# acoustic-warfare/beamforming-lk

Measured on AMD Instinct MI355X. Metric: heatmap frames/sec, higher is better.
Workload: dtype f32

## Files before the change

beamforming-lk_amd/csrc/das_fast.hip:

```cpp
#include "das_kernels.h"

#include <algorithm>
#include <atomic>

namespace awpu {

typedef float f2 __attribute__((ext_vector_type(2)));
typedef float f4 __attribute__((ext_vector_type(4)));
typedef float f4u __attribute__((ext_vector_type(4), aligned(4)));
typedef float f8 __attribute__((ext_vector_type(8)));

#define AWPU_AS4 __attribute__((address_space(4)))

typedef int i16 __attribute__((ext_vector_type(16)));

struct EntryGroup {
    i16 v;
    __device__ __forceinline__ float f(int k) const { return __int_as_float(v[4 * k + 0]); }
    __device__ __forceinline__ unsigned addr(int k) const { return (unsigned) v[4 * k + 1]; }
    __device__ __forceinline__ float g(int k) const { return __int_as_float(v[4 * k + 2]); }
};

template <int FPI>
struct Reads {
// ... 39 lines not shown
    issue_reads<FPI>(r1, e.addr(1), lane_base);
    issue_reads<FPI>(r2, e.addr(2), lane_base);
    issue_reads<FPI>(r3, e.addr(3), lane_base);
    accumulate<FPI>(acc, r0, e.f(0), e.g(0));
    accumulate<FPI>(acc, r1, e.f(1), e.g(1));
    accumulate<FPI>(acc, r2, e.f(2), e.g(2));
    accumulate<FPI>(acc, r3, e.f(3), e.g(3));
}

#include "das_fast_trip.inc"
static_assert(kFirStaticPlaneBytes == kFirStaticPlaneBytesHost, "das_kernels.h and tools/gen_trip_asm.py disagree on the FIR8 plane pitch");

template <int PPW, bool LOW = false>
__device__ __forceinline__ void sweep_chunk_trips(Acc<1> (&acc)[PPW], const FastEntry *lut, int pix0,
                                                  int usable_pad, int m0, int ng, unsigned lane_addr) {
    const int stride = usable_pad * (int) sizeof(FastEntry);
    if constexpr (PPW % 4 == 0 && LOW) {
#pragma unroll
        for (int q = 0; q < PPW; q += 4) {
            const void *row = lut + (size_t) (pix0 + q) * usable_pad + m0;
            sweep_quad_lo(acc[q].A[0], acc[q].Q[0], acc[q].C[0], acc[q].R[0],
                          acc[q + 1].A[0], acc[q + 1].Q[0], acc[q + 1].C[0], acc[q + 1].R[0],
                          acc[q + 2].A[0], acc[q + 2].Q[0], acc[q + 2].C[0], acc[q + 2].R[0],
                          acc[q + 3].A[0], acc[q + 3].Q[0], acc[q + 3].C[0], acc[q + 3].R[0], row, stride, ng, lane_addr);
        }
    } else if constexpr (PPW % 4 == 0) {
#pragma unroll
        for (int q = 0; q < PPW; q += 4) {
            const void *row = lut + (size_t) (pix0 + q) * usable_pad + m0;
            sweep_quad_hi(acc[q].A[0], acc[q].Q[0], acc[q].C[0], acc[q].R[0],
                          acc[q + 1].A[0], acc[q + 1].Q[0], acc[q + 1].C[0], acc[q + 1].R[0],
                          acc[q + 2].A[0], acc[q + 2].Q[0], acc[q + 2].C[0], acc[q + 2].R[0],
                          acc[q + 3].A[0], acc[q + 3].Q[0], acc[q + 3].C[0], acc[q + 3].R[0], row, stride, ng, lane_addr);
        }
    } else {
#pragma unroll
        for (int pp = 0; pp < PPW; pp++) {
            const void *row = lut + (size_t) (pix0 + pp) * usable_pad + m0;
            sweep_pixel_hi(acc[pp].A[0], acc[pp].Q[0], acc[pp].C[0], acc[pp].R[0], row, stride, ng, lane_addr);
        }
    }
}

template <int PPW, bool LOW = false>
__device__ __forceinline__ void sweep_chunk_stamped(Acc<1> (&acc)[PPW], const FastEntry *lut, int pix0,
                                                    int usable_pad, int m0, int ng, unsigned lane_addr,
                                                    unsigned &t_wait, unsigned &t_all) {
    static_assert(PPW % 4 == 0, "diagnostic build: quads only");
    const int stride = usable_pad * (int) sizeof(FastEntry);
#pragma unroll
    for (int q = 0; q < PPW; q += 4) {
        const void *row = lut + (size_t) (pix0 + q) * usable_pad + m0;
        unsigned dw = 0, da = 0;
        if constexpr (LOW) {
            sweep_quad_lo_stamped(acc[q].A[0], acc[q].Q[0], acc[q].C[0], acc[q].R[0],
                                  acc[q + 1].A[0], acc[q + 1].Q[0], acc[q + 1].C[0], acc[q + 1].R[0],
                                  acc[q + 2].A[0], acc[q + 2].Q[0], acc[q + 2].C[0], acc[q + 2].R[0],
                                  acc[q + 3].A[0], acc[q + 3].Q[0], acc[q + 3].C[0], acc[q + 3].R[0], row, stride, ng,
                                  lane_addr, dw, da);
        } else
        sweep_quad_stamped(acc[q].A[0], acc[q].Q[0], acc[q].C[0], acc[q].R[0],
                           acc[q + 1].A[0], acc[q + 1].Q[0], acc[q + 1].C[0], acc[q + 1].R[0],
                           acc[q + 2].A[0], acc[q + 2].Q[0], acc[q + 2].C[0], acc[q + 2].R[0],
                           acc[q + 3].A[0], acc[q + 3].Q[0], acc[q + 3].C[0], acc[q + 3].R[0], row, stride, ng,
                           lane_addr, dw, da);
        t_wait += dw;
        t_all += da;
    }
}

template <int CTRL, int ROW_MASK = 0xf>
__device__ __forceinline__ float dpp_take(float v) {
    return __builtin_bit_cast(float, __builtin_amdgcn_update_dpp(0, __builtin_bit_cast(int, v), CTRL, ROW_MASK, 0xf, false));
}
__device__ __forceinline__ float wave_sum(float v) {
    v += dpp_take<0xB1>(v);
    v += dpp_take<0x4E>(v);
    v += dpp_take<0x141>(v);
    v += dpp_take<0x140>(v);
    v += dpp_take<0x142, 0xa>(v);
    v += dpp_take<0x143, 0xc>(v);
    return __builtin_bit_cast(float, __builtin_amdgcn_readlane(__builtin_bit_cast(int, v), 63));
}

__device__ __forceinline__ float fold_halves(float a, float b) {
    asm volatile("s_nop 1\n\tv_permlane32_swap_b32 %0, %1\n\ts_nop 1" : "+v"(a), "+v"(b));
    return a + b;
}
__device__ __forceinline__ float fold_rows(float a, float b) {
    asm volatile("s_nop 1\n\tv_permlane16_swap_b32 %0, %1\n\ts_nop 1" : "+v"(a), "+v"(b));
    return a + b;
}
__device__ __forceinline__ float wave_sum8(float v0, float v1, float v2, float v3, float v4, float v5, float v6, float v7, int lane) {
    const float x = fold_rows(fold_halves(v0, v1), fold_halves(v2, v3));
    const float y = fold_rows(fold_halves(v4, v5), fold_halves(v6, v7));
    const float xs = x + dpp_take<0x128>(x), ys = y + dpp_take<0x128>(y);
    float z = (lane & 8) ? ys : xs;
    z += dpp_take<0xB1>(z);
    z += dpp_take<0x4E>(z);
    z += dpp_take<0x141>(z);
    return z;
}
__device__ __forceinline__ constexpr int kWaveSum8Value(int group) { return 4 * (group & 1) + (((group >> 1) & 1) << 1) + (group >> 2); }
__device__ __forceinline__ float wave_sum4(float v0, float v1, float v2, float v3) {
    float z = fold_rows(fold_halves(v0, v1), fold_halves(v2, v3));
    z += dpp_take<0xB1>(z);
    z += dpp_take<0x4E>(z);
    z += dpp_take<0x141>(z);
    z += dpp_take<0x140>(z);
    return z;
}
__device__ __forceinline__ constexpr int kWaveSum4Value(int row) { return ((row & 1) << 1) + (row >> 1); }

__device__ __forceinline__ void store_powers8(const f2 (&s)[4], const int (&pix)[4], const bool (&live)[4], int pair, int batch,
                                              int pixel_count, float norm, float *power, int lane) {
    const float total = wave_sum8(s[0].x, s[0].y, s[1].x, s[1].y, s[2].x, s[2].y, s[3].x, s[3].y, lane);
    const int value = kWaveSum8Value(lane >> 3), pp = value >> 1, frame = 2 * pair + (value & 1);
    const int p = pp == 0 ? pix[0] : pp == 1 ? pix[1] : pp == 2 ? pix[2] : pix[3];
    const bool on = pp == 0 ? live[0] : pp == 1 ? live[1] : pp == 2 ? live[2] : live[3];
    if ((lane & 7) == 0 && on && frame < batch) power[(size_t) frame * pixel_count + p] = total / norm;
}

__device__ __forceinline__ float sum8(float v) {
    v += dpp_take<0xB1>(v);
    v += dpp_take<0x4E>(v);
    v += dpp_take<0x141>(v);
    return v;
}
__device__ __forceinline__ float sum16(float v) {
    v = sum8(v);
    return v + dpp_take<0x140>(v);
}
__device__ __forceinline__ float sum32(float v) {
    v = sum16(v);
    return v + dpp_take<0x142, 0xa>(v);
}
template <int LPP>
__device__ __forceinline__ float sum_lanes(float v) {
    static_assert(LPP == 8 || LPP == 16 || LPP == 32, "groups of 8, 16 or 32 lanes");
    return LPP == 8 ? sum8(v) : LPP == 16 ? sum16(v) : sum32(v);
}
template <int LPP>
__device__ __forceinline__ constexpr int sum_lane_of(int group) {
    return LPP == 32 ? 32 * group + 16 : LPP * group;
}
__device__ __forceinline__ float lane_value(float v, int lane_index) {
    return __builtin_bit_cast(float, __builtin_amdgcn_readlane(__builtin_bit_cast(int, v), lane_index));
}

constexpr int kDppWaveRol1 = 0x134;
constexpr int kDppWaveRor1 = 0x13C;
template <int CTRL>
__device__ __forceinline__ float wave_rotate1(float v) {
    const int bits = __builtin_bit_cast(int, v);
    return __builtin_bit_cast(float, __builtin_amdgcn_update_dpp(bits, bits, CTRL, 0xf, 0xf, false));
}

__device__ __forceinline__ float finish_pixel(f2 A, f2 Q, f2 C, f2 R, float tail, int lane) {
    const float q_rot = wave_rotate1<kDppWaveRol1>(Q.x);
    const float r_rot = wave_rotate1<kDppWaveRol1>(R.x);
    const float q_next = lane == 63 ? r_rot : q_rot;
    const float r_next = lane == 63 ? tail : r_rot;
    const float o0 = A.x + Q.y;
    const float o1 = A.y + q_next;
    const float o2 = C.x + R.y;
    const float o3 = C.y + r_next;
    const float o1_prev = wave_rotate1<kDppWaveRor1>(o1);
    const float o2_next = wave_rotate1<kDppWaveRol1>(o2);
    const float o0_rot = wave_rotate1<kDppWaveRol1>(o0);
    const float o3_rot = wave_rotate1<kDppWaveRor1>(o3);
    const float o0_next = lane == 63 ? o2_next : o0_rot;
    const float o3_prev = lane == 0 ? o1_prev : o3_rot;
    const float ma0 = o0 * 0.5f - 0.25f * (o1 + o1_prev);
    const float ma1 = o1 * 0.5f - 0.25f * (o0_next + o0);
    const float ma2 = o2 * 0.5f - 0.25f * (o3 + o3_prev);
    const float ma3 = o3 * 0.5f - 0.25f * (o2_next + o2);
    float sum = ma1 * ma1 + ma2 * ma2;
    if (lane != 0) sum += ma0 * ma0;
    if (lane != 63) sum += ma3 * ma3;
    return wave_sum(sum);
}

template <int NW, int PPW, int FPI, int WPS>
__global__ __launch_bounds__(NW * 64, WPS) void das_fast_kernel(FastArgs a) {
    static_assert(PPW <= 8, "the tail pass gives 8 lanes to each of at most 8 pixels");
    extern __shared__ __attribute__((aligned(16))) float lds[];
    constexpr int FS = kFastLdsBytes / FPI;
    const int lane = threadIdx.x & 63;
    const int wave = __builtin_amdgcn_readfirstlane(threadIdx.x >> 6);
    const char *lane_base = (const char *) lds + lane * 8;
    const unsigned lane_addr = (unsigned) (unsigned long long) (const __attribute__((address_space(3))) char *) lane_base;
    const int frame0 = blockIdx.x * FPI;
    const int pix0 = (blockIdx.y * NW + wave) * PPW;
    const int wr = a.wr;
    const AWPU_AS4 FastEntry *lut = (const AWPU_AS4 FastEntry *) (unsigned long long) a.lut;
    const AWPU_AS4 int32_t *index = (const AWPU_AS4 int32_t *) (unsigned long long) a.index;
    const AWPU_AS4 int32_t *row_off = (const AWPU_AS4 int32_t *) (unsigned long long) a.row_off;

    Acc<FPI> acc[PPW];
    float tail[FPI];
#pragma unroll
    for (int b = 0; b < FPI; b++) tail[b] = 0.0f;
#pragma unroll
    for (int pp = 0; pp < PPW; pp++)
#pragma unroll
        for (int b = 0; b < FPI; b++) acc[pp].A[b] = acc[pp].Q[b] = acc[pp].C[b] = acc[pp].R[b] = f2{0.0f, 0.0f};

    constexpr int LPP = 8, NU = 32 / LPP;
    const int tail_pp = lane / LPP;
    const bool tail_lane = tail_pp < PPW && pix0 + tail_pp < a.pixel_count;
    const FastEntry *tail_row = a.lut + (size_t) (pix0 + (tail_lane ? tail_pp : 0)) * a.usable_pad;
    struct AddrG {
        unsigned addr;
        float g;
    };

    for (int m0 = 0; m0 < a.usable; m0 += a.chunk) {
        const int mc = min(a.chunk, a.usable - m0);
        const int mc4 = (mc + 3) & ~3;
        AddrG te[NU];
#pragma unroll
        for (int u = 0; u < NU; u++) {
            const int j = LPP * u + ((lane - m0) & (LPP - 1));
            te[u] = *(const AddrG *) ((const char *) (tail_row + m0 + min(j, mc4 - 1)) + 4);
            if (!tail_lane || j >= mc4) te[u].g = 0.0f;
        }
        __syncthreads();

        const int rows = AWPU_DBG(a, 1) && m0 > 0 ? 0 : FPI * mc * 2;
        const bool inside = a.wstart + 1 + wr <= a.hist;
        if (inside && !AWPU_DBG(a, 64)) {
            for (int r = wave; r < rows; r += NW) {
                const int b = r / (2 * mc);
                const int jr = r - b * 2 * mc;
                const int fb = min(frame0 + b, a.batch - 1);
                const float *src = a.frames + (size_t) fb * a.n_streams * a.hist + row_off[2 * m0 + jr];
                float *dst = lds + b * (FS / 4) + jr * wr;
                for (int t0 = 0; t0 < wr; t0 += 256) {
                    if (t0 + lane * 4 < wr) {
                        __builtin_amdgcn_global_load_lds((const __attribute__((address_space(1))) void *) (src + t0 + lane * 4),
                                                         (__attribute__((address_space(3))) void *) (dst + t0), 16, 0, 0);
                    }
                }
            }
            asm volatile("s_waitcnt vmcnt(0)" ::: "memory");
        } else
        for (int r = wave; r < rows; r += 2 * NW) {
            const float *src[2];
            float *dst[2];
            int valid[2];
#pragma unroll
            for (int u = 0; u < 2; u++) {
                const int rr = min(r + u * NW, rows - 1);
                const int b = rr / (2 * mc);
                const int jr = rr - b * 2 * mc;
                const int j = jr >> 1, q = jr & 1;
                const int fb = min(frame0 + b, a.batch - 1);
                const int first = a.wstart + q;
                src[u] = a.frames + ((size_t) fb * a.n_streams + index[m0 + j]) * a.hist + first;
                dst[u] = lds + b * (FS / 4) + (j * 2 + q) * wr;
                valid[u] = min(wr, a.hist - first);
            }
            if (valid[0] == wr && valid[1] == wr) {
                for (int t0 = 0; t0 < wr; t0 += 512) {
                    f4 v[2][2];
#pragma unroll
                    for (int u = 0; u < 2; u++)
#pragma unroll
                        for (int k = 0; k < 2; k++) {
                            const int t = t0 + k * 256 + lane * 4;
                            if (t < wr) v[u][k] = *(const f4u *) (src[u] + t);
                        }
#pragma unroll
                    for (int u = 0; u < 2; u++)
#pragma unroll
                        for (int k = 0; k < 2; k++) {
                            const int t = t0 + k * 256 + lane * 4;
                            if (t < wr) *(f4 *) (dst[u] + t) = v[u][k];
                        }
                }
            } else {
#pragma unroll
                for (int u = 0; u < 2; u++)
                    for (int t = lane; t < wr; t += 64) dst[u][t] = t < valid[u] ? src[u][t] : 0.0f;
            }
        }
        __syncthreads();

        if (!AWPU_DBG(a, 2)) {
            if constexpr (FPI == 1) {
                sweep_chunk_trips<PPW>(acc, a.lut, pix0, a.usable_pad, m0, mc4 >> 2, lane_addr);
            } else {
#pragma unroll
                for (int pp = 0; pp < PPW; pp++) {
                    const int p = pix0 + pp;
                    if (p < a.pixel_count) {
                        const AWPU_AS4 i16 *grp = (const AWPU_AS4 i16 *) (lut + (size_t) p * a.usable_pad + m0);
                        const int ng = mc4 >> 2;
                        EntryGroup e0, e1;
                        e0.v = grp[0];
                        for (int g = 0; g < ng; g += 2) {
                            e1.v = grp[g + 1];
                            sweep_group<FPI>(acc[pp], e0, lane_base);
                            e0.v = grp[g + 2];
                            if (g + 1 < ng) sweep_group<FPI>(acc[pp], e1, lane_base);
                        }
                    }
                }
// ... 119 lines not shown
        const int buf = step & 1;
        const bool last_chunk = c + 1 == n_chunks;
        const int c1 = last_chunk ? 0 : c + 1;
        const int fi1 = last_chunk ? fi + 1 : fi;
        long long t = diag ? __builtin_readcyclecounter() : 0;
        if (step + 1 < n_steps && !AWPU_DBG(a, 1)) {
            dma_chunk(frame0 + fi1, c1 * a.chunk, min(a.chunk, a.usable - c1 * a.chunk), buf ^ 1);
        }
        stamp(0, t);

        const unsigned lane_addr = lds_base + buf * BUF + lane * 8;
        if constexpr (DIAG) {
            sweep_chunk_stamped<PPW, (WPS > 4)>(acc, a.lut, pix0, a.usable_pad, m0, mc4 >> 2, lane_addr, t_wait, t_all);
        } else if (!AWPU_DBG(a, 2)) {
            sweep_chunk_trips<PPW, (WPS > 4)>(acc, a.lut, pix0, a.usable_pad, m0, mc4 >> 2, lane_addr);
        }
        stamp(1, t);
        const float *buf_f = lds + buf * (BUF / 4);
        for (int j0 = 0; j0 < (AWPU_DBG(a, 4) ? 0 : mc4); j0 += 32) {
            FastEntry e[4];
#pragma unroll
            for (int u = 0; u < 4; u++) {
                const int j = j0 + 8 * u + ((lane - m0) & 7);
                e[u] = tail_row[m0 + min(j, mc4 - 1)];
                if (!tail_lane || j >= mc4) e[u].g = 0.0f;
            }
#pragma unroll
            for (int u = 0; u < 4; u++) tail = __builtin_fmaf(e[u].g, buf_f[(e[u].addr + 1024u) >> 2], tail);
        }
        if (diag) asm volatile("s_waitcnt lgkmcnt(0)" ::: "memory");
        stamp(2, t);
        asm volatile("s_waitcnt vmcnt(0)" ::: "memory");
        stamp(3, t);
        if (!AWPU_DBG(a, 8)) __syncthreads();
        stamp(4, t);

        if (last_chunk) {
            tail = sum8(tail);
#pragma unroll
            for (int pp = 0; pp < PPW; pp++) {
                const int p = pix0 + pp;
                const float tl = lane_value(tail, pp * 8);
                const float sum = finish_pixel(acc[pp].A[0], acc[pp].Q[0], acc[pp].C[0], acc[pp].R[0], tl, lane);
                if (lane == 0 && p < a.pixel_count) {
                    a.power[(size_t) (frame0 + fi) * a.pixel_count + p] = sum / (float) (kSamples * a.usable);
                }
                acc[pp].A[0] = acc[pp].Q[0] = acc[pp].C[0] = acc[pp].R[0] = f2{0.0f, 0.0f};
            }
            tail = 0.0f;
        }
        c = c1;
        fi = fi1;
    }

    if (DIAG && a.debug_out && lane == 0) {
        unsigned long long *o = a.debug_out + 12 * ((size_t) (blockIdx.y * gridDim.x + blockIdx.x) * NW + wave);
        o[0] = t_wait;
        o[1] = t_all;
        o[2] = (unsigned long long) (__builtin_readcyclecounter() - t_begin);
        o[3] = (unsigned long long) n_steps * PPW;
        for (int k = 0; k < 5; k++) o[4 + k] = t_ph[k];
    }
}

template <bool FILTER>
__device__ __forceinline__ void pack_one_row(const float *frames, int n_streams, int hist, int wstart, const int32_t *index,
                                             int usable, const float *gain, int wp, int batch, float *packed, int pair, int s,
                                             int rows_out) {
    f2 *dst = (f2 *) packed + ((size_t) pair * rows_out + s) * wp;
    if (s >= usable) {
        for (int t = threadIdx.x; t < wp; t += blockDim.x) dst[t] = f2{0.0f, 0.0f};
        return;
    }
    const int fa = min(2 * pair, batch - 1), fb = min(2 * pair + 1, batch - 1);
    const float *xa = frames + ((size_t) fa * n_streams + index[s]) * hist + wstart;
    const float *xb = frames + ((size_t) fb * n_streams + index[s]) * hist + wstart;
    const float gm = gain ? gain[s] : 1.0f;
    const int valid = min(wp, hist - wstart);
    for (int t = threadIdx.x; t < wp; t += blockDim.x) {
        f2 v = f2{0.0f, 0.0f};
        if (t < valid) {
            v = f2{xa[t] * gm, xb[t] * gm};
            if constexpr (FILTER) {
                const bool lo = wstart + t > 0, hi = wstart + t + 1 < hist;
                const f2 nb = f2{(lo ? xa[t - 1] * gm : 0.0f) + (hi ? xa[t + 1] * gm : 0.0f),
                                 (lo ? xb[t - 1] * gm : 0.0f) + (hi ? xb[t + 1] * gm : 0.0f)};
                v = __builtin_elementwise_fma(f2{-0.25f, -0.25f}, nb, 0.5f * v);
            }
        }
        dst[t] = v;
    }
}

template <bool FILTER>
__global__ void pack_pairs_kernel(const float *frames, int n_streams, int hist, int wstart, const int32_t *index,
                                  int usable, const float *gain, int wp, int batch, float *packed) {
    pack_one_row<FILTER>(frames, n_streams, hist, wstart, index, usable, gain, wp, batch, packed, blockIdx.y, blockIdx.x, gridDim.x);
}

template <int CTRL>
__device__ __forceinline__ f2 wave_rotate(f2 v) {
    return f2{wave_rotate1<CTRL>(v.x), wave_rotate1<CTRL>(v.y)};
}

__device__ __forceinline__ f2 finish_pixel_pair(const f2 (&P)[8], f2 tail, int lane) {
    f2 o[4];
    f2 rq = wave_rotate<kDppWaveRol1>(P[4]);
#pragma unroll
    for (int k = 0; k < 4; k++) {
        const f2 rq_next = k < 3 ? wave_rotate<kDppWaveRol1>(P[k < 3 ? 5 + k : 7]) : tail;
        o[k] = P[k] + (lane == 63 ? rq_next : rq);
        rq = rq_next;
    }
    f2 sum = f2{0.0f, 0.0f};
    f2 dn = wave_rotate<kDppWaveRol1>(o[0]);
    f2 up_before = wave_rotate<kDppWaveRor1>(o[0]);
#pragma unroll
    for (int k = 0; k < 4; k++) {
        const f2 dn_after = k < 3 ? wave_rotate<kDppWaveRol1>(o[k < 3 ? k + 1 : 3]) : dn;
        const f2 up = wave_rotate<kDppWaveRor1>(o[k]);
        const f2 next = lane == 63 ? dn_after : dn;
        const f2 prev = lane == 0 ? up_before : up;
        const int i = lane + 64 * k;
        const f2 ma = o[k] * 0.5f - 0.25f * (next + prev);
        if (i >= 1 && i <= kSamples - 2) sum += ma * ma;
        dn = dn_after;
        up_before = up;
    }
    sum.x = wave_sum(sum.x);
    sum.y = wave_sum(sum.y);
    return sum;
}

__device__ __forceinline__ f2 pixel_pair_partial_filtered(const f2 (&P)[8], int lane) {
    f2 sum = f2{0.0f, 0.0f};
    f2 rq = wave_rotate<kDppWaveRol1>(P[4]);
#pragma unroll
    for (int k = 0; k < 4; k++) {
        const f2 rq_next = k < 3 ? wave_rotate<kDppWaveRol1>(P[k < 3 ? 5 + k : 7]) : rq;
        const f2 ma = P[k] + (lane == 63 ? rq_next : rq);
        const int i = lane + 64 * k;
        if (i >= 1 && i <= kSamples - 2) sum = __builtin_elementwise_fma(ma, ma, sum);
        rq = rq_next;
    }
    return sum;
}
__device__ __forceinline__ f2 finish_pixel_pair_filtered(const f2 (&P)[8], int lane) {
    f2 sum = pixel_pair_partial_filtered(P, lane);
    sum.x = wave_sum(sum.x);
    sum.y = wave_sum(sum.y);
    return sum;
}

__device__ __forceinline__ const void *uniform_ptr(const void *p) {
    const unsigned long long v = (unsigned long long) p;
    const unsigned lo = __builtin_amdgcn_readfirstlane((unsigned) v);
    const unsigned hi = __builtin_amdgcn_readfirstlane((unsigned) (v >> 32));
    return (const void *) (((unsigned long long) hi << 32) | lo);
}

template <int PPW, bool DIAG, bool SHARE>
__global__ __launch_bounds__(1024, 4) void das_pair_kernel(PairArgs a) {
    static_assert(PPW % 2 == 0 && PPW <= 8, "pixels go through the asm blocks two at a time");
    extern __shared__ __attribute__((aligned(16))) float lds[];
    constexpr int NW = 16, kThreads = NW * 64, BUF = kFastLdsBytes;
    constexpr int kPieces = (BUF + kThreads * 16 - 1) / (kThreads * 16);
    const int lane = threadIdx.x & 63;
    const int wave = __builtin_amdgcn_readfirstlane(threadIdx.x >> 6);
    const unsigned lds_base = (unsigned) (unsigned long long) (const __attribute__((address_space(3))) char *) lds;
    const int total = a.n_pairs * a.tiles;
    const int per_xcd = (total + 7) >> 3;
    const int item = (blockIdx.x & 7) * per_xcd + (blockIdx.x >> 3);
    if (item >= min(total, ((int) (blockIdx.x & 7) + 1) * per_xcd)) return;
    int pair, tile;
    {
        const int full_items = (a.n_pairs / a.pair_group) * a.pair_group * a.tiles;
        const int ga = item < full_items ? a.pair_group : a.n_pairs % a.pair_group;
        const int rem = item < full_items ? item : item - full_items;
        const int grp = rem / (a.tiles * ga), in = rem - grp * a.tiles * ga;
        tile = in / ga;
        pair = (item < full_items ? grp * a.pair_group : a.n_pairs - ga) + (in - tile * ga);
    }
    int pix[PPW];
    bool live[PPW];
    int pair_rows;
    if (a.cols > 0) {
        static_assert(PPW == 4, "vertical pairing: 2 columns x 2 rows per wave");
        const int tiles_per_rowpair = (a.cols + 2 * NW - 1) / (2 * NW);
        const int row2 = tile / tiles_per_rowpair, col0 = (tile - row2 * tiles_per_rowpair) * 2 * NW + 2 * wave;
        const int rows = a.pixel_count / a.cols;
#pragma unroll
        for (int q = 0; q < PPW; q++) {
            const int row = 2 * row2 + (q & 1), col = col0 + (q >> 1);
            live[q] = row < rows && col < a.cols;
            pix[q] = min(2 * row2 * a.cols + col, a.pixel_count - 1) + (q & 1) * a.cols;
        }
        pair_rows = a.cols;
    } else {
#pragma unroll
        for (int q = 0; q < PPW; q++) {
            pix[q] = (tile * NW + wave) * PPW + q;
            live[q] = pix[q] < a.pixel_count;
        }
        pair_rows = 1;
    }
    const size_t row_floats = (size_t) a.wp * 2;
    const float *pair_base = a.packed + (size_t) pair * a.usable * row_floats;

    f2 acc[PPW][8];
#pragma unroll
    for (int pp = 0; pp < PPW; pp++)
#pragma unroll
        for (int k = 0; k < 8; k++) acc[pp][k] = f2{0.0f, 0.0f};

    auto dma_chunk = [&](int m0, int mc, int buf) {
        const float *src = pair_base + (size_t) m0 * row_floats;
        const int n_pieces = (int) ((size_t) mc * row_floats / 4);
#pragma unroll
        for (int k = 0; k < kPieces; k++) {
            const int piece = threadIdx.x + k * kThreads;
            if (piece < n_pieces) {
                float *dst = lds + buf * (BUF / 4) + (wave * 64 + k * kThreads) * 4;
                __builtin_amdgcn_global_load_lds((const __attribute__((address_space(1))) void *) (src + (size_t) piece * 4),
                                                 (__attribute__((address_space(3))) void *) dst, 16, 0, 0);
            }
        }
    };

    unsigned t_wait = 0, t_all = 0;
    const long long t_begin = __builtin_readcyclecounter();
    const int n_chunks = (a.usable + a.chunk - 1) / a.chunk;
    dma_chunk(0, min(a.chunk, a.usable), 0);
    asm volatile("s_waitcnt vmcnt(0)" ::: "memory");
    __syncthreads();

    unsigned t_ph[5] = {0, 0, 0, 0, 0};
    auto stamp = [&](int k, long long &t) {
        if (DIAG) {
            const long long n = __builtin_readcyclecounter();
            t_ph[k] += (unsigned) (n - t);
            t = n;
        }
    };
    const int stride = pair_rows * a.usable_pad * (int) sizeof(FastEntry);
    const int rank = wave >> 2;
    for (int c = 0; c < n_chunks; c++) {
        const int m0 = c * a.chunk;
        const int mc = min(a.chunk, a.usable - m0);
        const int mc4 = (mc + 3) & ~3;
        const int buf = c & 1;
        long long t = DIAG ? __builtin_readcyclecounter() : 0;
        if (c + 1 < n_chunks && !AWPU_DBG(a, 1)) dma_chunk(m0 + a.chunk, min(a.chunk, a.usable - m0 - a.chunk), buf ^ 1);
        stamp(0, t);
        const unsigned lane_addr = lds_base + buf * BUF + lane * 8;
#pragma unroll
        for (int q = 0; q < PPW; q += 2) {
            const void *row = uniform_ptr(a.lut + (size_t) pix[q] * a.usable_pad + m0);
            const int ng = __builtin_amdgcn_readfirstlane(mc4 >> 2);
            if constexpr (DIAG) {
                unsigned dw = 0, da = 0;
                if constexpr (SHARE) sweep_duo_shared_stamped(acc[q], acc[q + 1], row, stride, ng, lane_addr, rank, dw, da);
                else sweep_duo_pairs_stamped(acc[q], acc[q + 1], row, stride, ng, lane_addr, rank, dw, da);
                t_wait += dw;
                t_all += da;
            } else {
                if constexpr (SHARE) sweep_duo_shared(acc[q], acc[q + 1], row, stride, ng, lane_addr, rank);
                else sweep_duo_pairs(acc[q], acc[q + 1], row, stride, ng, lane_addr, rank);
            }
        }
        stamp(1, t);
        if (DIAG) asm volatile("s_waitcnt lgkmcnt(0)" ::: "memory");
        stamp(2, t);
        asm volatile("s_waitcnt vmcnt(0)" ::: "memory");
        stamp(3, t);
        if (!AWPU_DBG(a, 8)) __syncthreads();
        stamp(4, t);
    }

    if (DIAG && a.debug_out && lane == 0) {
        unsigned long long *o = a.debug_out + 12 * ((size_t) item * NW + wave);
        o[0] = t_wait;
        o[1] = t_all;
        o[2] = (unsigned long long) (__builtin_readcyclecounter() - t_begin);
        o[3] = (unsigned long long) n_chunks * PPW;
        for (int k = 0; k < 5; k++) o[4 + k] = t_ph[k];
    }
    const float norm = (float) (kSamples * a.usable);
    static_assert(PPW == 4, "store_powers8: four pixels x two frames per wave");
    f2 part[PPW];
#pragma unroll
    for (int pp = 0; pp < PPW; pp++) {
        part[pp] = pixel_pair_partial_filtered(acc[pp], lane);
    }
    store_powers8(part, pix, live, pair, a.batch, a.pixel_count, norm, a.power, lane);
}


template <bool SHARE>
__global__ __launch_bounds__(1024, 4) void das_pair_stationary_kernel(PairArgs a, int n_tiles, int tiles_per_wg) {
    constexpr int PPW = 4;
    extern __shared__ __attribute__((aligned(16))) float lds[];
    constexpr int NW = 16, kThreads = NW * 64;
    const int lane = threadIdx.x & 63;
    const int wave = __builtin_amdgcn_readfirstlane(threadIdx.x >> 6);
    const unsigned lds_base = (unsigned) (unsigned long long) (const __attribute__((address_space(3))) char *) lds;
    const int pair = blockIdx.x;
// ... 251 lines not shown
    const float *pair_base = a.packed + (size_t) pair * a.usable_pad * row_floats;

    f8 O0 = {0, 0, 0, 0, 0, 0, 0, 0}, O1 = O0, O2 = O0, O3 = O0;

    auto dma_chunk = [&](int m0, int mc, int buf) {
        const float *src = pair_base + (size_t) m0 * row_floats;
        const int n_pieces = (int) ((size_t) mc * row_floats / 4);
#pragma unroll
        for (int k = 0; k < kPieces; k++) {
            const int piece = threadIdx.x + k * kThreads;
            if (piece < n_pieces) {
                float *dst = lds + buf * (BUF / 4) + (wave * 64 + k * kThreads) * 4;
                __builtin_amdgcn_global_load_lds((const __attribute__((address_space(1))) void *) (src + (size_t) piece * 4),
                                                 (__attribute__((address_space(3))) void *) dst, 16, 0, 0);
            }
        }
    };

    const int n_chunks = (a.usable_pad + a.chunk - 1) / a.chunk;
    dma_chunk(0, min(a.chunk, a.usable_pad), 0);
    asm volatile("s_waitcnt vmcnt(0)" ::: "memory");
    __syncthreads();
    const int rank = wave >> 2;
    for (int c = 0; c < n_chunks; c++) {
        const int m0 = c * a.chunk;
        const int mc = min(a.chunk, a.usable_pad - m0);
        const int buf = c & 1;
        if (c + 1 < n_chunks) dma_chunk(m0 + a.chunk, min(a.chunk, a.usable_pad - m0 - a.chunk), buf ^ 1);
        const unsigned lane_addr = lds_base + buf * BUF + lane * 8;
        const void *row = uniform_ptr(quad_lut + (size_t) (m0 >> 2) * 16);
        sweep_quad_exact(O0, O1, O2, O3, row, __builtin_amdgcn_readfirstlane(mc >> 2), lane_addr, rank);
        asm volatile("s_waitcnt vmcnt(0)" ::: "memory");
        __syncthreads();
    }

    const float norm = (float) (kSamples * a.usable);
    auto finish = [&](const f8 &O, int q) {
        const int row = 4 * row4 + q;
        const bool live = row < a.rows && col < a.cols;
        const int p = min(row, a.rows - 1) * a.cols + min(col, a.cols - 1);
        f2 o[4];
#pragma unroll
        for (int k = 0; k < 4; k++) o[k] = f2{O[2 * k], O[2 * k + 1]};
        if (a.sums && live) {
#pragma unroll
            for (int k = 0; k < 4; k++) {
                a.sums[((size_t) (2 * pair) * a.pixel_count + p) * kSamples + lane + 64 * k] = o[k].x;
                if (2 * pair + 1 < a.batch) a.sums[((size_t) (2 * pair + 1) * a.pixel_count + p) * kSamples + lane + 64 * k] = o[k].y;
            }
        }
        return pixel_pair_partial_exact(o, lane);
    };
    const f2 s0 = finish(O0, 0), s1 = finish(O1, 1), s2 = finish(O2, 2), s3 = finish(O3, 3);
    {
        const float total = wave_sum8(s0.x, s0.y, s1.x, s1.y, s2.x, s2.y, s3.x, s3.y, lane);
        const int value = kWaveSum8Value(lane >> 3), row = 4 * row4 + (value >> 1), frame = 2 * pair + (value & 1);
        if ((lane & 7) == 0 && row < a.rows && col < a.cols && frame < a.batch)
            a.power[(size_t) frame * a.pixel_count + (size_t) row * a.cols + col] = total / norm;
    }
}

__device__ __forceinline__ f2 next_and_difference(float cur, float next, float gm) {
#pragma clang fp contract(off)
    const float c = cur * gm, n = next * gm;
    return f2{n, c - n};
}

__global__ void pack_nd_kernel(const float *frames, int n_streams, int hist, int wstart, const int32_t *index, int usable,
                               const float *gain, int wq, int batch, float *packed) {
    const int pair = blockIdx.y, s = blockIdx.x, rows_out = gridDim.x;
    f4 *dst = (f4 *) packed + ((size_t) pair * rows_out + s) * wq;
    if (s >= usable) {
        for (int t = threadIdx.x; t < wq; t += blockDim.x) dst[t] = f4{0.0f, 0.0f, 0.0f, 0.0f};
        return;
    }
    const int fa = min(2 * pair, batch - 1), fb = min(2 * pair + 1, batch - 1);
    const float *xa = frames + ((size_t) fa * n_streams + index[s]) * hist + wstart;
    const float *xb = frames + ((size_t) fb * n_streams + index[s]) * hist + wstart;
    const float gm = gain ? gain[s] : 1.0f;
    const int valid = min(wq, hist - wstart - 1);
    for (int t = threadIdx.x; t < wq; t += blockDim.x) {
        f4 v = f4{0.0f, 0.0f, 0.0f, 0.0f};
        if (t < valid) {
            const f2 ea = next_and_difference(xa[t], xa[t + 1], gm), eb = next_and_difference(xb[t], xb[t + 1], gm);
            v = f4{ea.x, eb.x, ea.y, eb.y};
        }
        dst[t] = v;
    }
}

__global__ void nd_items_kernel(int2 *items, int n_pairs, int tiles, int pair_group, int tiles_per_row, int nq) {
    const int item = blockIdx.x * blockDim.x + threadIdx.x;
    if (item >= n_pairs * tiles) return;
    const int full_items = (n_pairs / pair_group) * pair_group * tiles;
    const int ga = item < full_items ? pair_group : n_pairs % pair_group;
    const int rem = item < full_items ? item : item - full_items;
    const int grp = rem / (tiles * ga), in = rem - grp * tiles * ga;
    const int tile = in / ga;
    const int pair = (item < full_items ? grp * pair_group : n_pairs - ga) + (in - tile * ga);
    const int rowq = tile / tiles_per_row, colt = tile - rowq * tiles_per_row;
    items[item] = int2{pair, (nq * rowq * tiles_per_row + colt) * 16};
}

struct NdQueues {
    unsigned *q;
    int per, total, tail;
    __device__ __forceinline__ int len(int x) const { return max(0, min(per, total - x * per)); }
    __device__ __forceinline__ int head(int x) const { return len(x) - min(len(x), tail); }
    __device__ __forceinline__ int take_head(int x) const {
        if (head(x) <= 0) return -1;
        const unsigned i = atomicAdd(&q[x], 1u);
        return i < (unsigned) head(x) ? x * per + (int) i : -1;
    }
    __device__ __forceinline__ int take_common() const {
        if (tail <= 0) return -1;
        for (;;) {
            const unsigned j = atomicAdd(&q[8], 1u);
            const int run = (int) (j / (unsigned) tail), k = (int) (j - (unsigned) run * (unsigned) tail);
            if (run >= 8) return -1;
            if (k < len(run) - head(run)) return run * per + head(run) + k;
        }
    }
    __device__ __forceinline__ int take(int xcd) const {
        int item = take_head(xcd);
        if (item < 0) item = take_common();
        for (int y = 1; item < 0 && y < 8; y++) item = take_head((xcd + y) & 7);
        return item;
    }
};

template <int NQ, bool SUMS>
__global__ __launch_bounds__(1024, 4) void das_exact_nd_kernel(ExactNdArgs a) {
    extern __shared__ __attribute__((aligned(16))) float lds[];
    constexpr int NW = 16, kThreads = NW * 64, BUF = kFastLdsBytes;
    constexpr int kPieces = (BUF + kThreads * 16 - 1) / (kThreads * 16);
    const int wave = __builtin_amdgcn_readfirstlane(threadIdx.x >> 6);
    const unsigned lds_base = (unsigned) (unsigned long long) (const __attribute__((address_space(3))) char *) lds;
    int *mail = (int *) (lds + 2 * (BUF / 4));
    const int total = a.n_pairs * a.tiles;
    unsigned xcc;
    asm volatile("s_getreg_b32 %0, hwreg(HW_REG_XCC_ID)" : "=s"(xcc));
    const NdQueues Q{a.queue, (total + 7) >> 3, total, a.tail};
    const int xcd = (int) (xcc & 7u);
    if (threadIdx.x == 0) {
        const int first = Q.take(xcd);
        mail[0] = first;
        mail[1] = first >= 0 ? Q.take(xcd) : -1;
    }
    __syncthreads();
    int cur = __builtin_amdgcn_readfirstlane(mail[0]), nxt = __builtin_amdgcn_readfirstlane(mail[1]);
    if (cur < 0) return;
    __syncthreads();

    auto decode = [&](int item, int &pair, int &tile_quad) {
        const int2 d = a.items[item];
        pair = __builtin_amdgcn_readfirstlane(d.x);
        tile_quad = __builtin_amdgcn_readfirstlane(d.y);
    };
    const int tiles_per_row = (a.cols + NW - 1) / NW;
    const int groups_total = a.usable_pad >> 2;
    const size_t row_floats = (size_t) a.wq * 4;
    const int n_chunks = (a.usable_pad + a.chunk - 1) / a.chunk;
    const int first_mics = min(a.chunk, a.usable_pad), last_mics = a.usable_pad - (n_chunks - 1) * a.chunk;
    const int ngf = __builtin_amdgcn_readfirstlane(first_mics >> 2), ngl = __builtin_amdgcn_readfirstlane(last_mics >> 2);
    const unsigned dbf = __builtin_amdgcn_readfirstlane((unsigned) ((size_t) a.chunk * row_floats * 4));
    const unsigned dbl = __builtin_amdgcn_readfirstlane((unsigned) ((size_t) last_mics * row_floats * 4));
    const unsigned db0 = __builtin_amdgcn_readfirstlane((unsigned) ((size_t) first_mics * row_floats * 4));
    const int rank = wave >> 2;
    const int own_head = Q.head(xcd);

    int pair, tile;
    decode(cur, pair, tile);
#ifdef AWPU_TUNING_BUILD
    const unsigned long long rt_begin = a.debug_out ? __builtin_amdgcn_s_memrealtime() : 0ull;
    long long t_sweep = 0, t_other = 0, t_mark = __builtin_readcyclecounter();
    int n_items = 0;
#endif
    {
        const float *pair_base = a.packed + (size_t) pair * a.usable_pad * row_floats;
        const int n_pieces = (int) ((size_t) first_mics * row_floats / 4);
#pragma unroll
        for (int k = 0; k < kPieces; k++) {
            const int piece = threadIdx.x + k * kThreads;
            if (piece < n_pieces) {
                float *dst = lds + (wave * 64 + k * kThreads) * 4;
                __builtin_amdgcn_global_load_lds((const __attribute__((address_space(1))) void *) (pair_base + (size_t) piece * 4),
                                                 (__attribute__((address_space(3))) void *) dst, 16, 0, 0);
            }
        }
    }
    asm volatile("s_waitcnt vmcnt(0)" ::: "memory");
    __syncthreads();
    unsigned step = 0;

    for (;;) {
        const int cols_pad = tiles_per_row * NW;
        const int rowq = tile / (NQ * cols_pad);
        const int col = tile - NQ * rowq * cols_pad + wave;
        const int quad0 = tile + wave;
        const QuadEntry *quad_lut = a.lut + (size_t) quad0 * groups_total * 16;
        const float *pair_base = a.packed + (size_t) pair * a.usable_pad * row_floats;
        int pair_next = pair, tile_next = tile;
        if (nxt >= 0) decode(nxt, pair_next, tile_next);
        const float *next_base = a.packed + (size_t) pair_next * a.usable_pad * row_floats;
        unsigned ticket = 0;
        const bool asked = wave == 0 && nxt >= 0 && own_head > 0;
        const unsigned *qptr = (const unsigned *) uniform_ptr(asked ? a.queue + xcd : nullptr);

        f8 O[NQ][4];
#ifdef AWPU_TUNING_BUILD
        { const long long n = __builtin_readcyclecounter(); t_other += n - t_mark; t_mark = n; }
#endif
        {
            unsigned tid = threadIdx.x;
            asm volatile("" : "+v"(tid));
            const unsigned lane_bytes = tid * 16;
            const int buf = (int) (step & 1);
            unsigned lane_addr = lds_base + buf * BUF + (tid & 63) * 16;
            const unsigned ddst = __builtin_amdgcn_readfirstlane(lds_base + (buf ^ 1) * BUF + wave * 1024);
            const int delta = __builtin_amdgcn_readfirstlane(buf ? -BUF : BUF);
            const unsigned dbn = __builtin_amdgcn_readfirstlane(nxt >= 0 ? db0 : 0u);
            if constexpr (NQ == 1) {
                sweep_exact_nd_item1(O[0][0], O[0][1], O[0][2], O[0][3], uniform_ptr(quad_lut), ngf, ngl, __builtin_amdgcn_readfirstlane(n_chunks),
                                     lane_addr, rank, uniform_ptr(pair_base), dbf, dbl, uniform_ptr(next_base), dbn, ddst, delta, lane_bytes, qptr, ticket);
            } else {
                static_assert(NQ == 2, "blocks are generated for one and two quads per wave");
                const int qstride = __builtin_amdgcn_readfirstlane(tiles_per_row * NW * groups_total * 16 * (int) sizeof(QuadEntry));
                sweep_exact_nd_item2(O[0][0], O[0][1], O[0][2], O[0][3], O[1][0], O[1][1], O[1][2], O[1][3], uniform_ptr(quad_lut), qstride, ngf, ngl,
                                     __builtin_amdgcn_readfirstlane(n_chunks), lane_addr, rank, uniform_ptr(pair_base), dbf, dbl, uniform_ptr(next_base),
                                     dbn, ddst, delta, lane_bytes, qptr, ticket);
            }
            step += n_chunks;
        }
        if (threadIdx.x == 0 && nxt >= 0) {
            int got = own_head > 0 && ticket < (unsigned) own_head ? xcd * Q.per + (int) ticket : -1;
            if (got < 0) {
                got = Q.take_common();
                for (int y = 1; got < 0 && y < 8; y++) got = Q.take_head((xcd + y) & 7);
            }
            mail[0] = got;
        }
#ifdef AWPU_TUNING_BUILD
        { const long long n = __builtin_readcyclecounter(); t_sweep += n - t_mark; t_mark = n; n_items++; }
#endif

        unsigned tid_e = threadIdx.x;
        asm volatile("" : "+v"(tid_e));
        const int lane = (int) (tid_e & 63);
        const float norm = (float) (kSamples * a.usable);
#pragma unroll
        for (int q = 0; q < NQ; q++) {
            const int row4 = NQ * rowq + q;
            auto finish = [&](const f8 &Op, int pp) {
                const int row = 4 * row4 + pp;
                const bool live = row < a.rows && col < a.cols;
                const int p = min(row, a.rows - 1) * a.cols + min(col, a.cols - 1);
                f2 o[4];
#pragma unroll
                for (int k = 0; k < 4; k++) o[k] = f2{Op[2 * k], Op[2 * k + 1]};
                if (SUMS && live) {
#pragma unroll
                    for (int k = 0; k < 4; k++) {
                        a.sums[((size_t) (2 * pair) * a.pixel_count + p) * kSamples + lane + 64 * k] = o[k].x;
                        if (2 * pair + 1 < a.batch) a.sums[((size_t) (2 * pair + 1) * a.pixel_count + p) * kSamples + lane + 64 * k] = o[k].y;
                    }
                }
                return pixel_pair_partial_exact(o, lane);
            };
            const f2 s0 = finish(O[q][0], 0), s1 = finish(O[q][1], 1), s2 = finish(O[q][2], 2), s3 = finish(O[q][3], 3);
            const float sum = wave_sum8(s0.x, s0.y, s1.x, s1.y, s2.x, s2.y, s3.x, s3.y, lane);
            const int value = kWaveSum8Value(lane >> 3), row = 4 * row4 + (value >> 1), frame = 2 * pair + (value & 1);
            if ((lane & 7) == 0 && row < a.rows && col < a.cols && frame < a.batch)
                a.power[(size_t) frame * a.pixel_count + (size_t) row * a.cols + col] = sum / norm;
        }

        if (nxt < 0) break;
        __syncthreads();
        cur = nxt;
        pair = pair_next;
        tile = tile_next;
        nxt = __builtin_amdgcn_readfirstlane(mail[0]);
        __syncthreads();
    }
#ifdef AWPU_TUNING_BUILD
    if (a.debug_out && threadIdx.x == 0) {
        unsigned hw_id;
        asm volatile("s_getreg_b32 %0, hwreg(HW_REG_HW_ID)" : "=s"(hw_id));
        unsigned long long *o = a.debug_out + 8 * (size_t) blockIdx.x;
        o[0] = rt_begin;
        o[1] = __builtin_amdgcn_s_memrealtime();
        o[2] = (unsigned long long) t_other;
        o[3] = (unsigned long long) t_sweep;
        o[4] = (unsigned long long) (__builtin_readcyclecounter() - t_mark);
        o[5] = ((unsigned long long) xcc << 32) | hw_id;
        o[6] = (unsigned long long) n_items;
        o[7] = 1;
    }
#endif
}

__device__ __forceinline__ void store_tile_and_signal(float *lds, bool holder, int tile_row, int wave, int lane, float value, float *power, int row0,
                                                      int col0, int rows, int cols, const DoneFlag &done) {
    __syncthreads();
    if (holder) lds[tile_row * 16 + wave] = value;
    __syncthreads();
    if (wave != 0) return;
    const int r = row0 + (lane >> 4), c = col0 + (lane & 15);
    if (r < rows && c < cols) __hip_atomic_store(&power[(size_t) r * cols + c], lds[lane], __ATOMIC_RELAXED, __HIP_MEMORY_SCOPE_SYSTEM);
    asm volatile("s_waitcnt vmcnt(0)" ::: "memory");
    if (lane == 0 && __hip_atomic_fetch_add(done.counter, 1ull, __ATOMIC_RELAXED, __HIP_MEMORY_SCOPE_AGENT) + 1ull == done.target)
        __hip_atomic_store(done.flag, done.seq, __ATOMIC_RELAXED, __HIP_MEMORY_SCOPE_SYSTEM);
}

__global__ void pack_ndh_kernel(const float *frames, int n_streams, int pitch, int wstart, const int32_t *index, int usable,
                                const float *gain, int wh, float *packed) {
    const int frame = blockIdx.y, s = blockIdx.x, rows_out = gridDim.x;
    f4 *dst = (f4 *) packed + ((size_t) frame * rows_out + s) * wh;
    if (s >= usable) {
        for (int t = threadIdx.x; t < wh; t += blockDim.x) dst[t] = f4{0.0f, 0.0f, 0.0f, 0.0f};
        return;
    }
    const float *x = frames + ((size_t) frame * n_streams + (index ? index[s] : s)) * pitch + wstart;
    const float gm = gain ? gain[s] : 1.0f;
    for (int t = threadIdx.x; t < wh; t += blockDim.x) {
        const f2 lo = next_and_difference(x[t], x[t + 1], gm), hi = next_and_difference(x[t + 128], x[t + 129], gm);
        dst[t] = f4{lo.x, hi.x, lo.y, hi.y};
    }
}

__device__ __forceinline__ float pixel_partial_exact(const float (&o)[4], int lane) {
    float sum = 0.0f;
    float dn = wave_rotate1<kDppWaveRol1>(o[0]);
    float up_before = wave_rotate1<kDppWaveRor1>(o[0]);
#pragma unroll
    for (int k = 0; k < 4; k++) {
        const float dn_after = k < 3 ? wave_rotate1<kDppWaveRol1>(o[k < 3 ? k + 1 : 3]) : dn;
        const float up = wave_rotate1<kDppWaveRor1>(o[k]);
        const float next = lane == 63 ? dn_after : dn;
        const float prev = lane == 0 ? up_before : up;
        const int i = lane + 64 * k;
        const float ma = o[k] * 0.5f - 0.25f * (next + prev);
        if (i >= 1 && i <= kSamples - 2) sum += ma * ma;
        dn = dn_after;
        up_before = up;
    }
    return sum;
}

template <int NQ, bool STATIONARY>
__global__ __launch_bounds__(1024) void das_exact_ndh_kernel(ExactNdhArgs a) {
    extern __shared__ __attribute__((aligned(16))) float lds[];
    constexpr int NW = 16, kThreads = NW * 64, BUF = kFastLdsBytes;
    const int lane = threadIdx.x & 63;
    const int wave = __builtin_amdgcn_readfirstlane(threadIdx.x >> 6);
    const unsigned lds_base = (unsigned) (unsigned long long) (const __attribute__((address_space(3))) char *) lds;
    const int frame = blockIdx.x / a.tiles, tile = blockIdx.x - frame * a.tiles;
    constexpr int tile_cols = NW * NQ;
    const int tiles_per_row4 = (a.cols + tile_cols - 1) / tile_cols;
    const int row4 = tile / tiles_per_row4;
    const int col0 = (tile - row4 * tiles_per_row4) * tile_cols + wave * NQ;
    const int groups_total = a.usable_pad >> 2;
    const QuadEntry *quad_lut = a.lut + ((size_t) row4 * a.lut_cols + col0) * groups_total * 16;
    const size_t row_floats = (size_t) a.wh * 4;

    int n_chunks = 1, first_mics = a.usable_pad, last_mics = a.usable_pad;
    const float *frame_rows = nullptr;
    if constexpr (STATIONARY) {
        const float *frame_base = a.frames + (size_t) frame * a.n_streams * a.pitch + a.wstart;
        const int stretches = (a.wh + 63) >> 6;
        const int units = ((a.usable_pad - wave + NW - 1) / NW) * stretches;
        int r = 0, st = 0;
        constexpr int kUnits = 12;
        for (int u0 = 0; u0 < units; u0 += kUnits) {
            float c0[kUnits], n0[kUnits], c1[kUnits], n1[kUnits], gm[kUnits];
            int slot[kUnits];
#pragma unroll
            for (int j = 0; j < kUnits; j++) {
                const int s = wave + NW * r, t = 64 * st + lane;
                const bool on = u0 + j < units && t < a.wh;
                slot[j] = on ? s * a.wh + t : -1;
                c0[j] = n0[j] = c1[j] = n1[j] = 0.0f;
                gm[j] = 1.0f;
                if (on && s < a.usable) {
                    const float *x = frame_base + (size_t) (a.identity ? s : a.index[s]) * a.pitch + t;
                    c0[j] = x[0], n0[j] = x[1], c1[j] = x[128], n1[j] = x[129];
                    if (a.gain) gm[j] = a.gain[s];
                }
                if (++st == stretches) st = 0, r++;
            }
#pragma unroll
            for (int j = 0; j < kUnits; j++) {
                if (slot[j] < 0) continue;
                const f2 lo = next_and_difference(c0[j], n0[j], gm[j]), hi = next_and_difference(c1[j], n1[j], gm[j]);
                ((f4 *) lds)[slot[j]] = f4{lo.x, hi.x, lo.y, hi.y};
            }
        }
        __syncthreads();
#ifdef AWPU_NDH_STAGE_ONLY
        if (lds[threadIdx.x] != 12345.678f) return;
#endif
    } else {
        constexpr int kPieces = (BUF + kThreads * 16 - 1) / (kThreads * 16);
        frame_rows = a.packed + (size_t) frame * a.usable_pad * row_floats;
        n_chunks = (a.usable_pad + a.chunk - 1) / a.chunk;
        first_mics = min(a.chunk, a.usable_pad);
        last_mics = a.usable_pad - (n_chunks - 1) * a.chunk;
        const int n_pieces = (int) ((size_t) first_mics * row_floats / 4);
#pragma unroll
        for (int k = 0; k < kPieces; k++) {
            const int piece = threadIdx.x + k * kThreads;
            if (piece < n_pieces) {
                float *dst = lds + (wave * 64 + k * kThreads) * 4;
                __builtin_amdgcn_global_load_lds((const __attribute__((address_space(1))) void *) (frame_rows + (size_t) piece * 4),
                                                 (__attribute__((address_space(3))) void *) dst, 16, 0, 0);
            }
        }
        asm volatile("s_waitcnt vmcnt(0)" ::: "memory");
        __syncthreads();
    }

    f4 O[NQ][4];
    {
        unsigned lane_addr = lds_base + lane * 16;
        const int ngf = __builtin_amdgcn_readfirstlane(first_mics >> 2), ngl = __builtin_amdgcn_readfirstlane(last_mics >> 2);
        const unsigned dbf = __builtin_amdgcn_readfirstlane((unsigned) ((size_t) a.chunk * row_floats * 4));
        const unsigned dbl = __builtin_amdgcn_readfirstlane((unsigned) ((size_t) last_mics * row_floats * 4));
        const unsigned ddst = __builtin_amdgcn_readfirstlane(lds_base + BUF + wave * 1024);
        const int rank = wave >> 2;
        const unsigned lane_bytes = threadIdx.x * 16;
        const void *isrc = uniform_ptr(STATIONARY ? (const void *) a.lut : (const void *) frame_rows);
        const unsigned *no_queue = (const unsigned *) uniform_ptr(nullptr);
        unsigned no_ticket;
        if constexpr (NQ == 1 && STATIONARY) {
            sweep_exact_ndh_resident1(O[0][0], O[0][1], O[0][2], O[0][3], uniform_ptr(quad_lut), ngf, ngl, __builtin_amdgcn_readfirstlane(n_chunks),
                                      lane_addr, rank, isrc, dbf, dbl, isrc, 0u, ddst, BUF, lane_bytes, no_queue, no_ticket);
// ... 1251 lines not shown
```

Baseline: 23610.

## Restructure work-queue handoff to one barrier per item and prefetch next item decode

Moves the queue take for the following item into the epilogue before a single __syncthreads and decodes that item ahead of time. This replaces the two barriers per loop iteration and takes the next item's decode off the critical path. It also reloads scalar arguments from the kernarg segment through address-space-4 pointers with register pins, and changes wave_rotate1's DPP to the bound_ctrl form with a zero old value. Together these rearrange the scalar and synchronisation schedule, and any mistake in the mailbox ordering could cause a race.

Result: no change. 23570 (-0.2%).

```diff
diff --git a/beamforming-lk_amd/csrc/das_fast.hip b/beamforming-lk_amd/csrc/das_fast.hip
--- a/beamforming-lk_amd/csrc/das_fast.hip
+++ b/beamforming-lk_amd/csrc/das_fast.hip
@@ -215,8 +215,7 @@
 constexpr int kDppWaveRor1 = 0x13C;
 template <int CTRL>
 __device__ __forceinline__ float wave_rotate1(float v) {
-    const int bits = __builtin_bit_cast(int, v);
-    return __builtin_bit_cast(float, __builtin_amdgcn_update_dpp(bits, bits, CTRL, 0xf, 0xf, false));
+    return __builtin_bit_cast(float, __builtin_amdgcn_update_dpp(0, __builtin_bit_cast(int, v), CTRL, 0xf, 0xf, true));
 }
 
 __device__ __forceinline__ float finish_pixel(f2 A, f2 Q, f2 C, f2 R, float tail, int lane) {
@@ -642,6 +641,11 @@
     return sum;
 }
 
+template <class T>
+__device__ __forceinline__ T *global_ptr(T *p) {
+    return (T *) (__attribute__((address_space(1))) T *) p;
+}
+
 __device__ __forceinline__ const void *uniform_ptr(const void *p) {
     const unsigned long long v = (unsigned long long) p;
     const unsigned lo = __builtin_amdgcn_readfirstlane((unsigned) v);
@@ -1199,10 +1203,13 @@
     if (cur < 0) return;
     __syncthreads();
 
+    const AWPU_AS4 ExactNdArgs *kernarg = (const AWPU_AS4 ExactNdArgs *) __builtin_amdgcn_kernarg_segment_ptr();
+    typedef int i2 __attribute__((ext_vector_type(2)));
+    const AWPU_AS4 i2 *item_list = (const AWPU_AS4 i2 *) (unsigned long long) a.items;
     auto decode = [&](int item, int &pair, int &tile_quad) {
-        const int2 d = a.items[item];
-        pair = __builtin_amdgcn_readfirstlane(d.x);
-        tile_quad = __builtin_amdgcn_readfirstlane(d.y);
+        const i2 d = item_list[item];
+        pair = d.x;
+        tile_quad = d.y;
     };
     const int tiles_per_row = (a.cols + NW - 1) / NW;
     const int groups_total = a.usable_pad >> 2;
@@ -1214,10 +1221,12 @@
     const unsigned dbl = __builtin_amdgcn_readfirstlane((unsigned) ((size_t) last_mics * row_floats * 4));
     const unsigned db0 = __builtin_amdgcn_readfirstlane((unsigned) ((size_t) first_mics * row_floats * 4));
     const int rank = wave >> 2;
-    const int own_head = Q.head(xcd);
+    const int own_head = Q.head(xcd), own_base = xcd * Q.per;
 
     int pair, tile;
     decode(cur, pair, tile);
+    int pair_next = pair, tile_next = tile;
+    if (nxt >= 0) decode(nxt, pair_next, tile_next);
 #ifdef AWPU_TUNING_BUILD
     const unsigned long long rt_begin = a.debug_out ? __builtin_amdgcn_s_memrealtime() : 0ull;
     long long t_sweep = 0, t_other = 0, t_mark = __builtin_readcyclecounter();
@@ -1241,14 +1250,9 @@
     unsigned step = 0;
 
     for (;;) {
-        const int cols_pad = tiles_per_row * NW;
-        const int rowq = tile / (NQ * cols_pad);
-        const int col = tile - NQ * rowq * cols_pad + wave;
         const int quad0 = tile + wave;
         const QuadEntry *quad_lut = a.lut + (size_t) quad0 * groups_total * 16;
         const float *pair_base = a.packed + (size_t) pair * a.usable_pad * row_floats;
-        int pair_next = pair, tile_next = tile;
-        if (nxt >= 0) decode(nxt, pair_next, tile_next);
         const float *next_base = a.packed + (size_t) pair_next * a.usable_pad * row_floats;
         unsigned ticket = 0;
         const bool asked = wave == 0 && nxt >= 0 && own_head > 0;
@@ -1279,55 +1283,79 @@
             }
             step += n_chunks;
         }
-        if (threadIdx.x == 0 && nxt >= 0) {
-            int got = own_head > 0 && ticket < (unsigned) own_head ? xcd * Q.per + (int) ticket : -1;
-            if (got < 0) {
-                got = Q.take_common();
-                for (int y = 1; got < 0 && y < 8; y++) got = Q.take_head((xcd + y) & 7);
-            }
-            mail[0] = got;
-        }
 #ifdef AWPU_TUNING_BUILD
         { const long long n = __builtin_readcyclecounter(); t_sweep += n - t_mark; t_mark = n; n_items++; }
 #endif
-
+        const AWPU_AS4 ExactNdArgs *e = kernarg;
+        asm volatile("" : "+s"(e));
+        int rows = e->rows, cols = e->cols, batch = e->batch, pixel_count = e->pixel_count, usable = e->usable;
+        float *power = global_ptr(e->power);
         unsigned tid_e = threadIdx.x;
         asm volatile("" : "+v"(tid_e));
+        int nxt_e = nxt;
+        asm volatile("" : "+s"(nxt_e));
+        auto arrived = [&] { asm volatile("" : "+s"(rows), "+s"(cols), "+s"(batch), "+s"(pixel_count), "+s"(usable), "+s"(power)); };
+        int after = -1, pair_after = 0, tile_after = 0;
+        if (nxt_e >= 0) {
+            if (tid_e == 0) {
+                int got = own_head > 0 && ticket < (unsigned) own_head ? own_base + (int) ticket : -1;
+                if (got < 0) {
+                    unsigned xcc_e;
+                    asm volatile("s_getreg_b32 %0, hwreg(HW_REG_XCC_ID)" : "=s"(xcc_e));
+                    const int total_e = e->n_pairs * e->tiles, xcd_e = (int) (xcc_e & 7u);
+                    const NdQueues Qe{global_ptr(e->queue), (total_e + 7) >> 3, total_e, e->tail};
+                    got = Qe.take_common();
+                    for (int y = 1; got < 0 && y < 8; y++) got = Qe.take_head((xcd_e + y) & 7);
+                }
+                mail[0] = got;
+            }
+            arrived();
+            __syncthreads();
+            after = __builtin_amdgcn_readfirstlane(mail[0]);
+            if (after >= 0) decode(after, pair_after, tile_after);
+        } else {
+            arrived();
+        }
+
+        const int cols_pad = (cols + NW - 1) / NW * NW;
+        const int rowq = tile / (NQ * cols_pad);
+        const int col = tile - NQ * rowq * cols_pad + wave;
         const int lane = (int) (tid_e & 63);
-        const float norm = (float) (kSamples * a.usable);
+        const float norm = (float) (kSamples * usable);
 #pragma unroll
         for (int q = 0; q < NQ; q++) {
-            const int row4 = NQ * rowq + q;
             auto finish = [&](const f8 &Op, int pp) {
-                const int row = 4 * row4 + pp;
-                const bool live = row < a.rows && col < a.cols;
-                const int p = min(row, a.rows - 1) * a.cols + min(col, a.cols - 1);
                 f2 o[4];
 #pragma unroll
                 for (int k = 0; k < 4; k++) o[k] = f2{Op[2 * k], Op[2 * k + 1]};
-                if (SUMS && live) {
-#pragma unroll
-                    for (int k = 0; k < 4; k++) {
-                        a.sums[((size_t) (2 * pair) * a.pixel_count + p) * kSamples + lane + 64 * k] = o[k].x;
-                        if (2 * pair + 1 < a.batch) a.sums[((size_t) (2 * pair + 1) * a.pixel_count + p) * kSamples + lane + 64 * k] = o[k].y;
+                if constexpr (SUMS) {
+                    const int row = 4 * (NQ * rowq + q) + pp;
+                    const int p = min(row, rows - 1) * cols + min(col, cols - 1);
+                    float *sums = global_ptr(e->sums);
+                    if (row < rows && col < cols) {
+#pragma unroll
+                        for (int k = 0; k < 4; k++) {
+                            sums[((size_t) (2 * pair) * pixel_count + p) * kSamples + lane + 64 * k] = o[k].x;
+                            if (2 * pair + 1 < batch) sums[((size_t) (2 * pair + 1) * pixel_count + p) * kSamples + lane + 64 * k] = o[k].y;
+                        }
                     }
                 }
                 return pixel_pair_partial_exact(o, lane);
             };
             const f2 s0 = finish(O[q][0], 0), s1 = finish(O[q][1], 1), s2 = finish(O[q][2], 2), s3 = finish(O[q][3], 3);
             const float sum = wave_sum8(s0.x, s0.y, s1.x, s1.y, s2.x, s2.y, s3.x, s3.y, lane);
-            const int value = kWaveSum8Value(lane >> 3), row = 4 * row4 + (value >> 1), frame = 2 * pair + (value & 1);
-            if ((lane & 7) == 0 && row < a.rows && col < a.cols && frame < a.batch)
-                a.power[(size_t) frame * a.pixel_count + (size_t) row * a.cols + col] = sum / norm;
+            const int value = kWaveSum8Value(lane >> 3), row = 4 * (NQ * rowq + q) + (value >> 1), frame = 2 * pair + (value & 1);
+            if ((lane & 7) == 0 && row < rows && col < cols && frame < batch)
+                power[(size_t) frame * pixel_count + (size_t) row * cols + col] = sum / norm;
         }
 
         if (nxt < 0) break;
-        __syncthreads();
         cur = nxt;
         pair = pair_next;
         tile = tile_next;
-        nxt = __builtin_amdgcn_readfirstlane(mail[0]);
-        __syncthreads();
+        nxt = after;
+        pair_next = after >= 0 ? pair_after : pair;
+        tile_next = after >= 0 ? tile_after : tile;
     }
 #ifdef AWPU_TUNING_BUILD
     if (a.debug_out && threadIdx.x == 0) {
```
